# exoplanet-dev/exoplanet

Measured on AMD Instinct MI355X. Metric: light-curve evals/sec (value+grad) at 150k cadences, higher is better.
Workload: dtype f64; 1 GPU; BASELINE configs[1] (C2): single planet e=0.3 Kepler solve + quadratic limb-darkened transit, 150000 cadences, value+grad, use_in_transit=False: dense flux output; n_cadences=150000, draws_per_gpu=1024, global_draws=1024, parallelism=draws sharded over 1 GPU(s); one collective of per-draw scalars per step

## Files before the change

### exoplanet_amd/csrc/exo_transit.hip

```cpp
#include <hip/hip_runtime.h>
#include <stdint.h>

#include "../../include/exoplanet_amd.h"
#include "exo_contact.hpp"
#include "exo_math.hpp"
#include "exo_pack_core.hpp"

namespace {

constexpr int kBlock = 256;
constexpr int kWaves = kBlock / 64;
constexpr int kTile = 2 * kBlock;
#ifndef EXO_TARGET_BLOCKS
#define EXO_TARGET_BLOCKS (256 * 16)
#endif
constexpr int kTargetBlocks = EXO_TARGET_BLOCKS;
constexpr uint32_t kFlagNoFluxDev = 0x80000000u;
constexpr int kNG = 12;
constexpr int kMaxMerge = 8;
constexpr int kWin = 7;
enum { G_N = 0, G_TP, G_ECC, G_COSW, G_SINW, G_COSI, G_AOR, G_ROR, G_FR, G_PAD, G_SINI, G_CL };
constexpr double kCLight = 37231.66360672704;

struct PlanetConst {
  double n, tp, e, se, pe, sq1me2, cw, sw, ci, si, aor, ror, iror;
  double t0, period, iperiod, ts, te, fr, ts2, te2, isq1me2;
  double clr;
  float ef, omf, sqf, cwf, swf, cif, zsf, thrf, zthrf, inthrf;
  double nrev, c0, dmid, half[2];
  double te0, tinv;
  int tfin;
};

struct Shared {
  PlanetConst pc[EXO_MAX_PLANETS];
  double c[6];
  double sdt[EXO_MAX_SUBEXP + 1];
  double sw[EXO_MAX_SUBEXP + 1];
  double red[16][16];
};

#ifndef EXO_WINDOW_REFINE
#define EXO_WINDOW_REFINE 1
#endif
constexpr int kSortBlock = 4096;
constexpr int kWinLanes = 8;
__device__ __forceinline__ void window_lanes(const double* __restrict__ p, uint32_t flags, int sub, double* w) {
  const int which = sub >> 2, k = (sub >> 1) & 1, sd = sub & 1;
  const double e = p[EXO_P_ECC], cw = p[EXO_P_COSW], sw = p[EXO_P_SINW];
  if (flags & EXO_FLAG_WINDOW) {
    const double ip = 1.0 / p[EXO_P_PERIOD];
    const double ts = p[EXO_P_TS], te = p[EXO_P_TE], ts2 = p[EXO_P_TS2], te2 = p[EXO_P_TE2];
    const bool fin = (fabs(ts) < __builtin_inf()) && (fabs(te) < __builtin_inf());
    const bool fin2 = (fabs(ts2) < __builtin_inf()) && (fabs(te2) < __builtin_inf());
    const double mid = fin ? 0.5 * (ts + te) : 0.0, mid2 = fin2 ? 0.5 * (ts2 + te2) : 0.0;
    w[0] = ip;
    w[1] = -(p[EXO_P_T0] + mid) * ip;
    w[2] = (mid - mid2) * ip;
    w[3] = fin ? fma(0.5 * (te - ts) * ip, 1.0 + 1e-12, 1e-14) : __builtin_inf();
    w[4] = fin2 ? fma(0.5 * (te2 - ts2) * ip, 1.0 + 1e-12, 1e-14) : __builtin_inf();
    const double wn_ = sqrt(cw * cw + sw * sw), r_ = fabs(p[EXO_P_ROR]);
    const double sinw_ = wn_ > 0.0 ? sw / wn_ : 0.0;
    for (int q = 0; q < 2; ++q) {
      const double bk = fabs(p[EXO_P_AOR] * p[EXO_P_COSI]) * (1.0 - e * e) / (1.0 + (q ? -e : e) * sinw_);
      const double in2 = (1.0 - r_) * (1.0 - r_) - bk * bk, out2 = (1.0 + r_) * (1.0 + r_) - bk * bk;
      const double h = w[3 + q];
      w[5 + q] = (r_ < 1.0 && in2 > 0.0 && out2 > 0.0 && h < __builtin_inf()) ? 0.95 * h * sqrt(in2 / out2) : 0.0;
    }
    if (flags & EXO_FLAG_LIGHT_DELAY) {
      const double vmax = fabs(p[EXO_P_N] * p[EXO_P_AOR]) * (1.0 + e) / sqrt(1.0 - e * e);
      const double dmax = fabs(p[EXO_P_AOR]) * (1.0 + e) / (fabs(p[EXO_P_CLIGHT]) - vmax);
      const double wd = (dmax >= 0.0 ? dmax : __builtin_inf()) * ip * 1.05;
      w[3] += wd; w[4] += wd;
    }
    return;
  }
  const double nrev = p[EXO_P_N] * (0.5 / exo::kPi);
  const double wn = sqrt(cw * cw + sw * sw);
  const double q = (1.0 + fabs(p[EXO_P_ROR])) / (fabs(p[EXO_P_AOR]) * (1.0 - e) * wn);
  const bool bounded = (e >= 0.0 && e < 1.0) && (q < 0.999);
  const bool want = bounded && (k == 0 || (flags & EXO_FLAG_SECONDARY));
  double m_pt = 0.0;
  bool has_in = false;
  if (want) {
    const double se = sqrt(1.0 - e), pe = sqrt(1.0 + e);
    const double s0 = p[EXO_P_SINI] < 0.0 ? -1.0 : 1.0, sk = k ? -1.0 : 1.0;
    const double sinw = sw / wn, cosw = cw / wn;
// ... 1374 lines not shown
    const double t_rate = (t_last - t_first) / (double)(n_cad > 1 ? n_cad - 1 : 1);
    for (int r = lane; r < K; r += 64) {
      int lo_k = 0, hi_k = nfin + 1;
      while (hi_k - lo_k > 1) {
        const int mid = (lo_k + hi_k) >> 1;
        if (s_first[mid] <= r) lo_k = mid; else hi_k = mid;
      }
      const int k = lo_k;
      const double kc = (double)(s_mlo[k] + (r - s_first[k]));
      const double sh = row.shift[k], off = -sh * nrev;
      auto first_not = [&](double thr, bool strict, int lo, int hi) {
        if (t_rate > 0.0 && hi > lo) {
          const double gq = ceil(((thr - c0) / nrev + sh - t_first) / t_rate);
          const int g = gq < (double)lo ? lo : (gq > (double)hi ? hi : (int)gq);
          const double xa = g > lo ? fma(t[g - 1], nrev, c0) + off : 0.0, xb = g < hi ? fma(t[g], nrev, c0) + off : 0.0;
          const bool left_before = g == lo || (strict ? (xa <= thr) : (xa < thr));
          const bool here_not = g == hi || !(strict ? (xb <= thr) : (xb < thr));
          if (left_before && here_not) return g;
        }
        while (lo < hi) {
          const int mid = (lo + hi) >> 1;
          const double xi = fma(t[mid], nrev, c0) + off;
          const bool before = strict ? (xi <= thr) : (xi < thr);
          lo = before ? mid + 1 : lo;
          hi = before ? hi : mid;
        }
        return lo;
      };
      Run q;
      q.lo = first_not(kc - h0, false, 0, (int)n_cad);
      q.hi = first_not(kc + h0, true, q.lo, (int)n_cad);
      if (hin > 0.0) {
        q.a = first_not(kc - hin, false, q.lo, q.hi);
        q.b = first_not(kc + hin, true, q.a, q.hi);
      } else {
        q.a = q.b = q.lo;
      }
      runs[r] = q;
      rbin[r] = k;
      s_len[0][r] = q.b - q.a;
      s_len[1][r] = q.hi - q.lo;
    }
  }
  __syncthreads();
  enum_prefix(s_len, K, lane, pin, pall, rl.nrun + list);
}

struct FillCursor {
  typedef double v2d __attribute__((ext_vector_type(2)));
  char* base;
  int64_t off;
  int left;
  uint32_t loff;
  v2d zero;
  __device__ __forceinline__ FillCursor(double* dst, int64_t n) : base(nullptr), off(0), left(0), loff((threadIdx.x & 63) * 16) {
    zero = v2d{0.0, 0.0};
    asm volatile("" : "+v"(zero));
    if (!dst || n <= 0) return;
    const int64_t head = (reinterpret_cast<uintptr_t>(dst) & 8) ? 1 : 0;
    if (threadIdx.x == 0 && head) dst[0] = 0.0;
    if (threadIdx.x == 0 && ((n - head) & 1)) dst[n - 1] = 0.0;
    v2d* q2 = reinterpret_cast<v2d*>(dst + head);
    const int64_t n2 = (n - head) >> 1;
    const int64_t nfull = n2 >> 6;
    const int rem = (int)(n2 & 63);
    if ((int)threadIdx.x < rem) __builtin_nontemporal_store(zero, q2 + (nfull << 6) + threadIdx.x);
    const int w = __builtin_amdgcn_readfirstlane((int)(threadIdx.x >> 6));
    left = nfull > w ? (int)((nfull - w + kWaves - 1) / kWaves) : 0;
    left = __builtin_amdgcn_readfirstlane(left);
    base = reinterpret_cast<char*>(q2);
    off = (int64_t)w * 1024;
  }
  __device__ __forceinline__ int pieces_left() const { return left; }
  __device__ __forceinline__ void issue(int count) {
    const int k = count < left ? count : left;
    for (int s = 0; s < k; ++s) {
      __builtin_nontemporal_store(zero, reinterpret_cast<v2d*>(base + off + loff));
      off += kWaves * 1024;
    }
    left -= k;
  }
};

__device__ __forceinline__ void finish_draw(
    int64_t draw, const double* partial, int nblk, int n_planet, bool secondary, double* __restrict__ gparams,
    double* __restrict__ gld, double* __restrict__ flux_dot, int64_t n_cad, uint32_t flags, int n_ev, const RunLists& rl,
    const double* vals, const int32_t* vcad, double* flux,
    const double* __restrict__ chi2_part, int n_chi2_part, double* __restrict__ chi2_out, const Ttv& ttv,
    int64_t cm_draws = 0) {
  if (ttv.gshift) {
    for (int p = 0; p < n_planet; ++p) {
      const int64_t list = draw * n_planet + p;
      const int K = rl.nrun[list];
      const int32_t* __restrict__ rbin = rl.rbin + list * rl.r_max;
      if (K == 0 || rbin[0] < 0) continue;
      const double* grun = rl.grun + list * rl.r_max;
      double* __restrict__ dst = ttv.gshift + list * (int64_t)(ttv.n_edge + 1);
      for (int k = threadIdx.x; k <= ttv.n_edge; k += (int)blockDim.x) {
        int lo = 0, hi = K;
        while (lo < hi) {
          const int mid = (lo + hi) >> 1;
          if (rbin[mid] < k) lo = mid + 1; else hi = mid;
        }
        double v = 0.0;
        for (int r = lo; r < K && rbin[r] == k; ++r) v += grun[r];
        dst[k] = v;
      }
    }
  }
  if (chi2_out && threadIdx.x == blockDim.x - 1) {
    double v = 0.0;
    for (int b = 0; b < n_chi2_part; ++b) v += chi2_part[draw * n_chi2_part + b];
    chi2_out[draw] = v;
  }
  const int ng_draw = n_planet * kNG + 7;
  const int s = threadIdx.x;
  if (partial) {
    for (int q = s; q < n_planet * EXO_NPAR; q += (int)blockDim.x) {
      const int p = q / EXO_NPAR, slot = q % EXO_NPAR;
      const bool carried = slot == EXO_P_N || slot == EXO_P_TP || slot == EXO_P_ECC || slot == EXO_P_COSW ||
                           slot == EXO_P_SINW || slot == EXO_P_COSI || slot == EXO_P_AOR || slot == EXO_P_ROR ||
                           slot == EXO_P_FRATIO || slot == EXO_P_SINI || slot == EXO_P_CLIGHT;
      if (!carried) gparams[(draw * n_planet + p) * EXO_NPAR + slot] = 0.0;
    }
    if (s < ng_draw) {
      const double* src = partial + draw * nblk * (int64_t)ng_draw + s;
      double v = 0.0;
      for (int b = 0; b < nblk; ++b) v += src[(int64_t)b * ng_draw];
      if (s < n_planet * kNG) {
        const int p = s / kNG, k = s % kNG;
        const int map[kNG] = {EXO_P_N, EXO_P_TP, EXO_P_ECC, EXO_P_COSW, EXO_P_SINW,
                              EXO_P_COSI, EXO_P_AOR, EXO_P_ROR, EXO_P_FRATIO, -1, EXO_P_SINI, EXO_P_CLIGHT};
        if (map[k] >= 0) gparams[(draw * n_planet + p) * EXO_NPAR + map[k]] = v;
      } else {
        const int k = s - n_planet * kNG;
        const int nld = secondary ? 6 : 3;
        if (k < nld) gld[draw * nld + k] = v;
        if (k == 6 && flux_dot) flux_dot[draw] = v;
      }
    }
  }
  if (!flux || !vals) return;
  const bool per_planet = flags & EXO_FLAG_PER_PLANET;
  const int nthr = (int)blockDim.x;
  __shared__ int s_total[EXO_MAX_PLANETS];
  if ((int)threadIdx.x < n_planet) {
    int total = 0;
    for (int ev = 0; ev < n_ev; ++ev) {
      const int64_t list = (draw * n_planet + threadIdx.x) * n_ev + ev;
      total += rl.pre_all[list * (rl.r_max + 1) + rl.nrun[list]];
    }
    s_total[threadIdx.x] = total;
  }
  __syncthreads();
  auto total_of = [&](int p) { return s_total[p]; };
  auto load = [&](int p, int cb, int total, double* v, int* i) {
    const int64_t vbase = (draw * n_planet + p) * n_cad;
#pragma unroll
    for (int u = 0; u < 4; ++u) {
      const int e = cb + (int)threadIdx.x + u * nthr;
      v[u] = e < total ? vals[vbase + e] : 0.0;
      i[u] = e < total ? vcad[vbase + e] : -1;
    }
  };
  int pl = 0, cb = -4 * nthr, total = total_of(0);
  auto advance = [&](int& p, int& c, int& tot) {
    c += 4 * nthr;
    while (p < n_planet && c >= tot) {
      ++p; c = 0;
      tot = p < n_planet ? total_of(p) : 0;
    }
  };
  advance(pl, cb, total);
  if (pl >= n_planet) return;
  double v[4];
  int i[4];
  load(pl, cb, total, v, i);
  for (;;) {
    int np = pl, ncb = cb, ntotal = total;
    advance(np, ncb, ntotal);
    const bool more = np < n_planet;
    double nv[4] = {0.0, 0.0, 0.0, 0.0};
    int ni[4] = {-1, -1, -1, -1};
    if (more) load(np, ncb, ntotal, nv, ni);
#pragma unroll
    for (int u = 0; u < 4; ++u) {
      if (i[u] < 0) continue;
      if (per_planet) {
        flux[(draw * n_cad + i[u]) * n_planet + pl] = v[u];
      } else {
        double* dst = cm_draws ? flux + (int64_t)i[u] * cm_draws + draw : flux + draw * n_cad + i[u];
        if (pl == 0) *dst = v[u]; else unsafeAtomicAdd(dst, v[u]);
      }
    }
    if (!more) break;
    if (!per_planet && np != pl) __syncthreads();
    pl = np; cb = ncb; total = ntotal;
#pragma unroll
    for (int u = 0; u < 4; ++u) { v[u] = nv[u]; i[u] = ni[u]; }
  }
}

__global__ __launch_bounds__(1024) void transit_finish_kernel(
    const double* __restrict__ partial, int nblk, int n_planet, bool secondary, double* __restrict__ gparams,
    double* __restrict__ gld, double* __restrict__ flux_dot, int64_t n_cad, uint32_t flags, int n_ev, RunLists rl,
    const double* __restrict__ vals, const int32_t* __restrict__ vcad, double* __restrict__ flux,
    const double* __restrict__ chi2_part, int n_chi2_part, double* __restrict__ chi2_out,
    Ttv ttv = Ttv{nullptr, nullptr, nullptr, 0}) {
  finish_draw(blockIdx.x, partial, nblk, n_planet, secondary, gparams, gld, flux_dot, n_cad, flags, n_ev, rl, vals, vcad, flux,
              chi2_part, n_chi2_part, chi2_out, ttv,
              ((flags & EXO_FLAG_CADENCE_MAJOR) && !(flags & EXO_FLAG_PER_PLANET)) ? (int64_t)gridDim.x : 0);
}

struct FinishArgs {
  double* gparams;
  double* gld;
  double* flux_dot;
  int fold;
  int32_t* done;
};

#ifndef EXO_RUNS_MIN_WAVES
#define EXO_RUNS_MIN_WAVES 3
#endif
constexpr int kJac = 16;
__device__ __forceinline__ int jac_slot(int s) {
  return s < G_PAD ? s : (s == G_SINI ? 9 : (s >= kNG && s < kNG + 6 ? 10 + (s - kNG) : -1));
}
template <bool GRAD, bool SECONDARY, bool LDELAY = false, bool CHI2 = false, bool TTV = false, bool JAC = false>
__global__ __launch_bounds__(kBlock, LDELAY ? 2 : EXO_RUNS_MIN_WAVES) void transit_runs_kernel(
    const double* __restrict__ t, int64_t n_cad, const double* __restrict__ texp, int64_t n_texp,
    const double* __restrict__ stencil_dt, const double* __restrict__ stencil_w, int n_sub,
    const double* __restrict__ params, const double* __restrict__ ld, int n_planet, uint32_t flags, int n_ev, RunLists rl,
    const double* __restrict__ gflux, const double* __restrict__ gsparse, double* __restrict__ vals,
    int32_t* __restrict__ vcad, double* __restrict__ fill, double* __restrict__ partial, int64_t chi2_nw = 0,
    Ttv ttv = Ttv{nullptr, nullptr, nullptr, 0}, FinishArgs fin = FinishArgs{nullptr, nullptr, nullptr, 0, nullptr}) {
  __shared__ Shared sh;
  __shared__ Run s_run[kSeg];
  __shared__ int2 s_pre[kSeg + 1];
  __shared__ int s_all[kSeg + 1];
  __shared__ int s_bin[TTV ? kSeg : 1];
  __shared__ double s_shift[TTV ? kSeg : 1];
  __shared__ double s_grun[(TTV && GRAD) ? kWaves : 1][(TTV && GRAD) ? kSeg : 1];
  __shared__ int s_rounds[2 * EXO_MAX_PLANETS];
  __shared__ double lds_acc[kNG + 7][kBlock];
  const int64_t draw = blockIdx.y;
  const int hb = gridDim.x, bx = blockIdx.x;
  stage_constants(sh, params, ld, stencil_dt, stencil_w, n_sub, n_planet, draw, SECONDARY);
  const bool per_planet = flags & EXO_FLAG_PER_PLANET;
  const int n_lists = n_planet * n_ev;
  auto slice = [&](int K, int& k0, int& k1) {
    k0 = (int)((int64_t)K * bx / hb);
    k1 = (int)((int64_t)K * (bx + 1) / hb);
  };
  if ((int)threadIdx.x < n_lists) {
    const int64_t list = draw * n_lists + threadIdx.x;
    int k0, k1;
    slice(rl.nrun[list], k0, k1);
    const int32_t* pall = rl.pre_all + list * (rl.r_max + 1);
    int rounds = 0;
    for (int kb = k0; kb < k1; kb += kSeg) {
      const int ke = (kb + kSeg < k1) ? kb + kSeg : k1;
      rounds += (pall[ke] - pall[kb] + kBlock - 1) / kBlock;
    }
    s_rounds[threadIdx.x] = rounds;
  }
  __syncthreads();
  int total_rounds = 0;
  for (int l = 0; l < n_lists; ++l) total_rounds += s_rounds[l];
  const int64_t npl = per_planet ? n_planet : 1, n_fill = n_cad * npl;
  const int64_t f0 = n_fill * bx / hb, f1 = n_fill * (bx + 1) / hb;
  FillCursor fc(fill ? fill + draw * n_fill + f0 : nullptr, f1 - f0);
  const int per_round =
      __builtin_amdgcn_readfirstlane(total_rounds > 0 ? (fc.pieces_left() + total_rounds - 1) / total_rounds : 0);

  static_assert(!JAC || (GRAD && !LDELAY && !CHI2 && !TTV), "the Jacobian sweep is the plain value + gradient evaluation");
  const int ng_draw = n_planet * kNG + 7;
  double* __restrict__ pout = (GRAD && !JAC) ? partial + ((int64_t)draw * hb + bx) * ng_draw : nullptr;
  double* __restrict__ jac = JAC ? partial : nullptr;
  const GradAcc acc{GRAD ? &lds_acc[0][threadIdx.x] : nullptr};
  if (GRAD) {
#pragma unroll
    for (int s = 0; s < kNG + 7; ++s) lds_acc[s][threadIdx.x] = 0.0;
  }
  double cld[6];
#pragma unroll
  for (int k = 0; k < 6; ++k) cld[k] = uniform((SECONDARY || k < 3) ? sh.c[k] : 0.0);
  const double te = (n_texp == 0) ? 0.0 : texp[0];
  const double sdt0 = uniform(sh.sdt[0]), sw0 = uniform(sh.sw[0]);
  for (int p = 0; p < n_planet; ++p) {
    const PlanetS c(sh.pc[p]);
    if (GRAD && p > 0) {
#pragma unroll
      for (int s = 0; s < kNG; ++s) lds_acc[s][threadIdx.x] = 0.0;
    }
    int64_t vbase = (draw * n_planet + p) * n_cad;
    const TtvRow row(ttv, TTV ? draw * n_planet + p : 0);
    double* __restrict__ grow = (TTV && GRAD) ? ttv.gshift + (draw * n_planet + p) * (int64_t)(ttv.n_edge + 1) : nullptr;
    const TtvGrad tgrad{(GRAD && TTV) ? &lds_acc[0][threadIdx.x] : nullptr, grow, nullptr};
    for (int ev = 0; ev < n_ev; ++ev) {
      const int64_t list = (draw * n_planet + p) * n_ev + ev;
      const int K = rl.nrun[list];
      const Run* __restrict__ runs = rl.runs + list * rl.r_max;
      const int32_t* __restrict__ pin = rl.pre_in + list * (rl.r_max + 1);
      const int32_t* __restrict__ pall = rl.pre_all + list * (rl.r_max + 1);
      int k0, k1;
      slice(K, k0, k1);
      for (int kb = k0; kb < k1; kb += kSeg) {
        const int m = (kb + kSeg < k1) ? kSeg : k1 - kb;
        __syncthreads();
        const int in0 = pin[kb], all0 = pall[kb];
        for (int q = threadIdx.x; q <= m; q += kBlock) {
          const int pi = pin[kb + q] - in0, pa = pall[kb + q];
          s_pre[q] = make_int2(pi, (pa - all0) - pi);
          s_all[q] = pa;
          if (q < m) s_run[q] = runs[kb + q];
          if (TTV && q < m) {
            const int kq = rl.rbin[list * rl.r_max + kb + q];
            s_bin[q] = kq;
            s_shift[q] = kq >= 0 ? row.shift[kq] : 0.0;
            if (GRAD) {
#pragma unroll
              for (int w = 0; w < kWaves; ++w) s_grun[w][q] = 0.0;
            }
          }
        }
        __syncthreads();
        const bool trusted = TTV && s_bin[0] >= 0;
        const int tin = s_pre[m].x, total = tin + s_pre[m].y;
        const float g_in = tin > 0 ? (float)m / (float)tin : 0.0f;
        const float g_lim = total > tin ? (float)m / (float)(total - tin) : 0.0f;
        struct Item { int i, v, q; double tv, g, w; };
        auto locate = [&](int j, int& i, int& v, int& qrun) {
          const bool in = j < tin;
          const int jj = in ? j : j - tin;
          int q = (int)((float)jj * (in ? g_in : g_lim));
          q = q < m - 1 ? q : m - 1;
          int2 pa = s_pre[q], pb = s_pre[q + 1];
          int lo = in ? pa.x : pa.y, hi = in ? pb.x : pb.y;
          int tries = 0;
          while (EXO_WAVE_ANY((jj < lo) | (jj >= hi))) {
            if (++tries > 4) {
              q = 0;
#pragma unroll
              for (int step = kSeg / 2; step > 0; step >>= 1) {
                const int c2 = q + step;
                if (c2 < m) {
                  const int2 pc = s_pre[c2];
                  q = (jj >= (in ? pc.x : pc.y)) ? c2 : q;
                }
              }
              pa = s_pre[q];
              lo = in ? pa.x : pa.y;
              break;
            }
            q += (jj < lo) ? -1 : ((jj >= hi) ? 1 : 0);
            pa = s_pre[q]; pb = s_pre[q + 1];
            lo = in ? pa.x : pa.y; hi = in ? pb.x : pb.y;
          }
          const Run r = s_run[q];
          const int off = jj - lo;
          i = in ? r.a + off : ((off < r.a - r.lo) ? r.lo + off : r.b + (off - (r.a - r.lo)));
          v = s_all[q] + (i - r.lo);
          qrun = q;
        };
        auto load_item = [&](int j) -> Item {
          Item it{0, 0, 0, 0.0, 0.0, 0.0};
          if (j < total) locate(j, it.i, it.v, it.q);
          it.tv = t[it.i];
          if (JAC) {
            it.g = (j < total) ? 1.0 : 0.0;
          } else if (CHI2) {
            if (j < total) { it.g = gflux[it.i]; it.w = gsparse[chi2_nw == 1 ? 0 : it.i]; }
          } else if (GRAD && j < total)
            it.g = gsparse ? gsparse[vbase + it.v]
                           : (per_planet ? gflux[(draw * n_cad + it.i) * n_planet + p]
                                         : ((flags & EXO_FLAG_CADENCE_MAJOR) ? gflux[(int64_t)it.i * gridDim.y + draw]
                                                                             : gflux[draw * n_cad + it.i]));
          return it;
        };
        Item nxt = load_item(threadIdx.x);
        for (int j0 = 0; j0 < total; j0 += kBlock) {
          const int j = j0 + threadIdx.x;
          const bool has = j < total;
          const Item cur = nxt;
          if (j0 + kBlock < total) nxt = load_item(j + kBlock);
          fc.issue(per_round);
          double f = 0.0;
          const double dsh = TTV ? s_shift[TTV ? cur.q : 0] : 0.0;
          for (int k = 0; k < n_sub; ++k) {
            const double sdt_k = (k == 0) ? sdt0 : sh.sdt[k], sw_k = (k == 0) ? sw0 : sh.sw[k];
            double tt = fma(te, sdt_k, cur.tv);
            int ks = 0;
            if (TTV) {
              double sh_k = dsh;
              if (!trusted) {
                ks = row.bin(tt);
                sh_k = row.shift[ks];
              }
              tt -= sh_k;
            }
            const double gw = cur.g * sw_k;
            const double F = eval_sample<GRAD, SECONDARY, LDELAY, CHI2>(tt, c, cld, CHI2 ? cur.g : gw, acc, cur.w);
            f = fma(sw_k, F, f);
            if (CHI2) {
              const double r = F - cur.g;
              acc.add(kNG + 6, cur.w * (r * r - cur.g * cur.g));
            } else if (GRAD && !JAC) {
              acc.add(kNG + 6, gw * F);
            }
            if (TTV && GRAD && !trusted) tgrad.flush_lane(ks);
          }
          if (TTV && GRAD && trusted) tgrad.flush_runs(cur.q, &s_grun[0][0], kSeg);
          if (JAC) {
            double row[kJac];
#pragma unroll
            for (int q = 0; q < kJac; ++q) row[q] = 0.0;
#pragma unroll
            for (int sl = 0; sl < kNG + 6; ++sl) {
              if (jac_slot(sl) >= 0) {
                row[jac_slot(sl)] = lds_acc[sl][threadIdx.x];
                lds_acc[sl][threadIdx.x] = 0.0;
              }
            }
            if (has) {
              double2* __restrict__ dst = reinterpret_cast<double2*>(jac + (vbase + cur.v) * kJac);
#pragma unroll
              for (int q = 0; q < kJac / 2; ++q) dst[q] = make_double2(row[2 * q], row[2 * q + 1]);
            }
          }
          if (vals && has) {
            vals[vbase + cur.v] = f;
            if (vcad) vcad[vbase + cur.v] = cur.i;
          }
        }
        if (TTV && GRAD && trusted) {
          __syncthreads();
          for (int q = threadIdx.x; q < m; q += kBlock) {
            double v = s_grun[0][q];
#pragma unroll
            for (int w = 1; w < kWaves; ++w) v += s_grun[(TTV && GRAD) ? w : 0][q];
            rl.grun[list * rl.r_max + kb + q] = v;
          }
        }
      }
      vbase += pall[K];
    }
    if (GRAD && TTV) {
      lds_acc[G_TP][threadIdx.x] = lds_acc[G_PAD][threadIdx.x];
      lds_acc[G_PAD][threadIdx.x] = 0.0;
    }
    if (GRAD && !JAC) reduce_columns(lds_acc, sh.red, 0, kNG, pout + p * kNG);
  }
  if (GRAD && !JAC) reduce_columns(lds_acc, sh.red, kNG, 7, pout + n_planet * kNG);
  fc.issue(1 << 30);
  if (fin.fold) {
    __syncthreads();
    finish_draw(draw, (GRAD && !JAC) ? partial : nullptr, hb, n_planet, SECONDARY, fin.gparams, fin.gld, fin.flux_dot, n_cad, flags, n_ev,
                rl, vals, vcad, fill, nullptr, 0, nullptr,
                (TTV && GRAD) ? ttv : Ttv{nullptr, nullptr, nullptr, 0});
  }
}

__global__ __launch_bounds__(kBlock) void transit_jac_vjp_kernel(int64_t n_cad, int n_planet, int n_ev, uint32_t flags,
                                                                 RunLists rl, const double* __restrict__ vals,
                                                                 const int32_t* __restrict__ vcad,
                                                                 const double* __restrict__ jac,
                                                                 const double* __restrict__ gflux, int64_t n_draw,
                                                                 double* __restrict__ partial) {
  __shared__ double red[kJac + 1][kBlock];
  const int64_t draw = blockIdx.y;
  const int nb = gridDim.x, bx = blockIdx.x;
  const int ng_draw = n_planet * kNG + 7;
  double* __restrict__ pout = partial + (draw * nb + bx) * ng_draw;
  const bool cmaj = flags & EXO_FLAG_CADENCE_MAJOR, gsp = flags & EXO_FLAG_SPARSE;
  double keep = 0.0;
  for (int p = 0; p < n_planet; ++p) {
    int n_vals = 0;
    for (int ev = 0; ev < n_ev; ++ev) {
      const int64_t list = (draw * n_planet + p) * n_ev + ev;
      n_vals += rl.pre_all[list * (rl.r_max + 1) + rl.nrun[list]];
    }
    const int64_t vbase = (draw * n_planet + p) * n_cad;
    double acc[kJac + 1];
#pragma unroll
    for (int q = 0; q <= kJac; ++q) acc[q] = 0.0;
    const int v0 = (int)((int64_t)n_vals * bx / nb), v1 = (int)((int64_t)n_vals * (bx + 1) / nb);
    for (int v = v0 + threadIdx.x; v < v1; v += kBlock) {
      double g;
      if (gsp) {
        g = gflux[vbase + v];
      } else {
        const int64_t i = vcad[vbase + v];
        g = cmaj ? gflux[i * n_draw + draw] : gflux[draw * n_cad + i];
      }
      const double2* __restrict__ row = reinterpret_cast<const double2*>(jac + (vbase + v) * kJac);
#pragma unroll
      for (int q = 0; q < kJac / 2; ++q) {
        const double2 r2 = row[q];
        acc[2 * q] = fma(g, r2.x, acc[2 * q]);
        acc[2 * q + 1] = fma(g, r2.y, acc[2 * q + 1]);
      }
      acc[kJac] = fma(g, vals[vbase + v], acc[kJac]);
    }
    __syncthreads();
#pragma unroll
    for (int q = 0; q <= kJac; ++q) red[q][threadIdx.x] = acc[q];
    __syncthreads();
    if (threadIdx.x <= kJac) {
      double v = 0.0;
      for (int k = 0; k < kBlock; ++k) v += red[threadIdx.x][k];
      const int q = threadIdx.x;
      if (q < 10) {
        pout[p * kNG + (q < 9 ? q : G_SINI)] = v;
      } else {
        keep += v;
      }
    }
    if (threadIdx.x < kNG && (threadIdx.x == G_PAD || threadIdx.x == G_CL)) pout[p * kNG + threadIdx.x] = 0.0;
  }
  if (threadIdx.x >= 10 && threadIdx.x <= kJac) pout[n_planet * kNG + (threadIdx.x - 10)] = keep;
}

constexpr int kResidualBlocks = 16;
__global__ __launch_bounds__(kBlock) void transit_residual_kernel(int64_t n_cad, int n_planet, int n_ev, RunLists rl,
                                                                  const double* __restrict__ vals,
                                                                  const int32_t* __restrict__ vcad,
                                                                  const double* __restrict__ obs,
                                                                  const double* __restrict__ ivar, int64_t n_ivar,
                                                                  double* __restrict__ gvals,
                                                                  double* __restrict__ chi2_part) {
  __shared__ double red[kBlock];
  const int64_t draw = blockIdx.y;
  const int nb = gridDim.x, n_lists = n_planet * n_ev;
  double acc = 0.0;
  auto lookup = [&](int l2, int i, bool& hit) -> double {
    const int64_t list = draw * n_lists + l2;
    const int K = rl.nrun[list];
    const Run* __restrict__ runs = rl.runs + list * rl.r_max;
    int lo = 0, hi = K;
    while (lo < hi) {
      const int mid = (lo + hi) >> 1;
// ... 118 lines not shown
  int64_t n_classify;
  dim3 grid;
};
inline ScanPlan scan_plan(uint32_t flags, int bpd, int64_t n_draw, int n_planet, int64_t n_texp, bool with_fill) {
  ScanPlan sp;
  const bool stage1 = (flags & EXO_FLAG_WINDOW) || !(flags & EXO_FLAG_EXACT_SCAN);
  const bool grouped = n_planet == 1 && n_texp <= 1 && stage1;
  sp.flags = (flags & 0x0fffffffu) | (grouped ? kFlagGrouped : 0u) | (with_fill ? 0u : kFlagNoFlux);
  sp.n_classify = (grouped ? (n_draw + kScanDraws - 1) / kScanDraws : n_draw) * bpd;
  sp.grid = dim3((unsigned)(sp.n_classify + (with_fill ? n_draw * bpd : 0)));
  return sp;
}

#ifndef EXO_RUNS_TARGET_BLOCKS
#define EXO_RUNS_TARGET_BLOCKS 512
#endif
inline int runs_blocks_per_draw(int64_t n_draw) {
  int64_t hb = (EXO_RUNS_TARGET_BLOCKS + n_draw - 1) / n_draw;
  return (int)(hb < 1 ? 1 : (hb > 64 ? 64 : hb));
}
inline int runs_r_max(int64_t n_cad) { return (int)(n_cad < kRunMax ? (n_cad < 16 ? 16 : n_cad) : kRunMax); }

struct RunWs {
  double* partial;
  double* windows;
  int32_t* sorted;
  RunLists rl;
  double* vals;
  int32_t* vcad;
  double* gvals;
  double* chi2_part;
  int32_t* done;
  int hb, n_sorted;
  int64_t off_nrun, off_runs, off_pre_all, off_vals;
  int64_t bytes;
};
inline RunWs carve_runs(void* base, int64_t n_cad, int64_t n_draw, int n_planet) {
  RunWs w;
  w.hb = runs_blocks_per_draw(n_draw);
  w.n_sorted = (int)((n_cad + kSortBlock - 1) / kSortBlock);
  w.rl.r_max = runs_r_max(n_cad);
  const int64_t n_list = n_draw * n_planet * 2;
  auto up16 = [](int64_t b) { return (b + 15) & ~(int64_t)15; };
  char* p = (char*)base;
  int64_t off = 0;
  w.partial = (double*)(p + off); off = up16(off + 8 * n_draw * w.hb * (int64_t)(n_planet * kNG + 7));
  w.windows = (double*)(p + off); off = up16(off + 8 * (int64_t)kWin * n_draw * n_planet);
  w.sorted = (int32_t*)(p + off); off = up16(off + 4 * (int64_t)w.n_sorted);
  w.off_nrun = off; w.rl.nrun = (int32_t*)(p + off); off = up16(off + 4 * n_list);
  w.off_runs = off; w.rl.runs = (Run*)(p + off); off = up16(off + (int64_t)sizeof(Run) * n_list * w.rl.r_max);
  w.rl.pre_in = (int32_t*)(p + off); off = up16(off + 4 * n_list * (int64_t)(w.rl.r_max + 1));
  w.off_pre_all = off; w.rl.pre_all = (int32_t*)(p + off); off = up16(off + 4 * n_list * (int64_t)(w.rl.r_max + 1));
  w.rl.rbin = (int32_t*)(p + off); off = up16(off + 4 * n_draw * n_planet * (int64_t)w.rl.r_max);
  w.rl.grun = (double*)(p + off); off = up16(off + 8 * n_draw * n_planet * (int64_t)w.rl.r_max);
  w.off_vals = off; w.vals = (double*)(p + off); off = up16(off + 8 * n_draw * n_planet * n_cad);
  w.vcad = (int32_t*)(p + off); off = up16(off + 4 * n_draw * n_planet * n_cad);
  w.gvals = (double*)(p + off); off = up16(off + 8 * n_draw * n_planet * n_cad);
  w.chi2_part = (double*)(p + off); off = up16(off + 8 * n_draw * kResidualBlocks);
  w.done = (int32_t*)(p + off); off = up16(off + 4 * n_draw);
  w.bytes = off;
  return w;
}
inline bool runs_path(bool has_ttv, int64_t n_texp, uint32_t flags) {
  if (has_ttv && (flags & (EXO_FLAG_SECONDARY | EXO_FLAG_LIGHT_DELAY))) return false;
  return n_texp <= 1 && !(flags & EXO_FLAG_EXACT_SCAN);
}

struct Chi2Args {
  const double* obs;
  const double* ivar;
  int64_t n_ivar;
  double* chi2;
};
struct RunsCommon {
  dim3 grid;
  hipStream_t st;
  const double *t, *texp, *stencil_dt, *stencil_w, *params, *ld;
  int64_t n_cad, n_texp;
  int n_sub, n_planet, n_ev;
  uint32_t flags;
  RunLists rl;
  Ttv ttv;
};
template <bool G, bool SEC, bool LDELAY = false, bool CHI2 = false, bool TTV = false, bool JAC = false>
inline void launch_runs(const RunsCommon& a, const double* gflux, const double* gsparse, double* vals, int32_t* vcad, double* fill,
                        double* partial, const FinishArgs& fin, int64_t chi2_nw = 0) {
  hipLaunchKernelGGL((transit_runs_kernel<G, SEC, LDELAY, CHI2, TTV, JAC>), a.grid, dim3(kBlock), 0, a.st, a.t, a.n_cad, a.texp,
                     a.n_texp, a.stencil_dt, a.stencil_w, a.n_sub, a.params, a.ld, a.n_planet, a.flags, a.n_ev, a.rl, gflux, gsparse,
                     vals, vcad, fill, partial, chi2_nw, a.ttv, fin);
}
inline int launch_runs_sweep(const double* t, int64_t n_cad, const double* texp, int64_t n_texp, const double* stencil_dt,
                             const double* stencil_w, int32_t n_sub, const double* params, const double* ld,
                             int64_t n_draw, int32_t n_planet, uint32_t flags, const double* gflux, double* flux,
                             double* gparams, double* gld, double* flux_dot, const RunWs& w, hipStream_t st,
                             const Chi2Args* chi2 = nullptr, const Ttv* ttv = nullptr, double* jac = nullptr,
                             const double* gvals = nullptr, bool reuse_runs = false, const PackIn* pack = nullptr) {
  const bool secondary = flags & EXO_FLAG_SECONDARY, sparse = (flags & EXO_FLAG_SPARSE) || chi2;
  const bool grad = gflux != nullptr || chi2 || gvals != nullptr;
  const int n_ev = secondary ? 2 : 1;
  const dim3 block(kBlock);
  const bool has_ttv = ttv && ttv->edges;
  const bool fused_enum = (flags & EXO_FLAG_SORTED_TIMES) && !has_ttv;
  if (reuse_runs) {
  } else if (!fused_enum) {
    const int64_t n_rec = n_draw * n_planet;
    hipLaunchKernelGGL(transit_window_kernel, dim3((unsigned)((n_rec * kWinLanes + kBlock - 1) / kBlock + w.n_sorted)), block, 0, st,
                       params, n_rec, flags, w.windows, t, n_cad, w.sorted, w.done, n_draw);
  }
  if (pack && (!fused_enum || reuse_runs)) return EXO_ERR_INVALID_ARGUMENT;
  if (reuse_runs) {
  } else if (pack) {
    const PackIn pk = *pack;
    hipLaunchKernelGGL((transit_enum_kernel<true, true>), dim3((unsigned)(n_draw * n_planet * n_ev)), dim3(64), 0, st, t, n_cad, texp,
                       n_texp, stencil_dt, (int)n_sub, flags, (const double*)nullptr, (const int32_t*)nullptr, 0, n_ev, w.rl,
                       params, w.windows, pk);
  } else if (fused_enum)
    hipLaunchKernelGGL(transit_enum_kernel<true>, dim3((unsigned)(n_draw * n_planet * n_ev)), dim3(64), 0, st, t, n_cad, texp,
                       n_texp, stencil_dt, (int)n_sub, flags, (const double*)nullptr, (const int32_t*)nullptr, 0, n_ev, w.rl,
                       params, w.windows);
  else if (has_ttv)
    hipLaunchKernelGGL(transit_enum_ttv_kernel, dim3((unsigned)(n_draw * n_planet)), dim3(64), 0, st, t, n_cad, texp, n_texp,
                       stencil_dt, (int)n_sub, flags, w.windows, w.sorted, w.n_sorted, w.rl, *ttv);
  else
    hipLaunchKernelGGL(transit_enum_kernel<false>, dim3((unsigned)(n_draw * n_planet * n_ev)), dim3(64), 0, st, t, n_cad, texp,
                       n_texp, stencil_dt, (int)n_sub, flags, w.windows, w.sorted, w.n_sorted, n_ev, w.rl);
  if (launch_status() != EXO_OK) return EXO_ERR_LAUNCH;
  double* vals = (flux || sparse) ? w.vals : nullptr;
  double* fill = sparse ? nullptr : flux;
  const bool ldelay = flags & EXO_FLAG_LIGHT_DELAY;
  const Ttv no_ttv{nullptr, nullptr, nullptr, 0};
  const RunsCommon ra{dim3((unsigned)w.hb, (unsigned)n_draw), st, t, texp, stencil_dt, stencil_w, params, ld, n_cad, n_texp, (int)n_sub,
                      (int)n_planet, n_ev, flags, w.rl, has_ttv ? *ttv : no_ttv};
  const bool cmaj = flags & EXO_FLAG_CADENCE_MAJOR;
  const bool fold = !(cmaj && flux) && w.hb == 1;
  const FinishArgs fin{gparams, gld, chi2 ? chi2->chi2 : flux_dot, fold ? 1 : 0, w.done}, no_fin{nullptr, nullptr, nullptr, 0, nullptr};
  auto plain = [&](auto g, const double* gf, const double* gsp, double* v, int32_t* vc, double* fl, double* part, const FinishArgs& f) {
    exo::with_flag(secondary, [&](auto sec) {
      exo::with_flag(ldelay, [&](auto ldl) {
        launch_runs<decltype(g)::value, decltype(sec)::value, decltype(ldl)::value>(ra, gf, gsp, v, vc, fl, part, f);
      });
    });
  };
  if (chi2 && n_planet == 1 && !secondary && n_sub == 1) {
    if (has_ttv)
      launch_runs<true, false, false, true, true>(ra, chi2->obs, chi2->ivar, nullptr, nullptr, nullptr, w.partial, fin, chi2->n_ivar);
    else if (ldelay)
      launch_runs<true, false, true, true>(ra, chi2->obs, chi2->ivar, nullptr, nullptr, nullptr, w.partial, fin, chi2->n_ivar);
    else
      launch_runs<true, false, false, true>(ra, chi2->obs, chi2->ivar, nullptr, nullptr, nullptr, w.partial, fin, chi2->n_ivar);
    if (launch_status() != EXO_OK) return EXO_ERR_LAUNCH;
    if (fold) return EXO_OK;
    hipLaunchKernelGGL(transit_finish_kernel, dim3((unsigned)n_draw), dim3(n_draw <= 256 ? 1024 : kBlock), 0, st, w.partial, w.hb,
                       (int)n_planet, secondary, gparams, gld, chi2->chi2, n_cad, flags, n_ev, w.rl, nullptr, w.vcad, nullptr,
                       nullptr, 0, nullptr, ra.ttv);
    return launch_status();
  }
  if (has_ttv && chi2) {
    launch_runs<false, false, false, false, true>(ra, nullptr, nullptr, w.vals, w.vcad, nullptr, nullptr, no_fin);
    hipLaunchKernelGGL(transit_residual_kernel, dim3(kResidualBlocks, (unsigned)n_draw), block, 0, st, n_cad, (int)n_planet,
                       n_ev, w.rl, w.vals, w.vcad, chi2->obs, chi2->ivar, chi2->n_ivar, w.gvals, w.chi2_part);
    launch_runs<true, false, false, false, true>(ra, nullptr, w.gvals, nullptr, nullptr, nullptr, w.partial, no_fin);
  } else if (has_ttv) {
    if (grad)
      launch_runs<true, false, false, false, true>(ra, gflux, nullptr, vals, fill ? w.vcad : nullptr, fill, w.partial, fin);
    else
      launch_runs<false, false, false, false, true>(ra, nullptr, nullptr, vals, fill ? w.vcad : nullptr, fill, nullptr, fin);
  } else if (chi2) {
    plain(std::false_type{}, nullptr, nullptr, w.vals, w.vcad, nullptr, nullptr, no_fin);
    hipLaunchKernelGGL(transit_residual_kernel, dim3(kResidualBlocks, (unsigned)n_draw), block, 0, st, n_cad, (int)n_planet,
                       n_ev, w.rl, w.vals, w.vcad, chi2->obs, chi2->ivar, chi2->n_ivar, w.gvals, w.chi2_part);
    plain(std::true_type{}, nullptr, w.gvals, nullptr, nullptr, nullptr, w.partial, no_fin);
  } else if (gvals) {
    plain(std::true_type{}, nullptr, gvals, nullptr, nullptr, nullptr, w.partial, fin);
  } else if (grad) {
    plain(std::true_type{}, gflux, nullptr, vals, fill ? w.vcad : nullptr, fill, w.partial, fin);
  } else if (jac) {
    exo::with_flag(secondary, [&](auto sec) {
      launch_runs<true, decltype(sec)::value, false, false, false, true>(ra, nullptr, nullptr, vals, w.vcad, fill, jac, fin);
    });
  } else {
    plain(std::false_type{}, nullptr, nullptr, vals, fill ? w.vcad : nullptr, fill, nullptr, fin);
  }
  if (launch_status() != EXO_OK) return EXO_ERR_LAUNCH;
  const bool three_sweeps = chi2 != nullptr;
  if ((grad || fill) && (!fold || three_sweeps))
    hipLaunchKernelGGL(transit_finish_kernel, dim3((unsigned)n_draw), dim3(n_draw <= 256 ? 1024 : kBlock), 0, st,
                       grad ? w.partial : nullptr, w.hb, (int)n_planet, secondary, gparams, gld, flux_dot, n_cad, flags, n_ev,
                       w.rl, chi2 ? nullptr : vals, w.vcad, fill, chi2 ? w.chi2_part : nullptr, kResidualBlocks,
                       chi2 ? chi2->chi2 : nullptr, grad ? ra.ttv : no_ttv);
  return launch_status();
}

template <bool CLEAR>
__global__ __launch_bounds__(kBlock) void transit_scatter_runs_kernel(RunLists rl, const double* __restrict__ vals, int64_t n_cad,
                                                                      int n_planet, int n_ev, double* __restrict__ flux) {
  const int64_t draw = blockIdx.x;
  const int wave = threadIdx.x >> 6, lane = threadIdx.x & 63, n_wave = kBlock / 64;
  double* __restrict__ row = flux + draw * n_cad;
  for (int p = 0; p < n_planet; ++p) {
    int64_t vbase = (draw * n_planet + p) * n_cad;
    for (int ev = 0; ev < n_ev; ++ev) {
      const int64_t list = (draw * n_planet + p) * n_ev + ev;
      int K = rl.nrun[list];
      K = K < 0 ? 0 : (K > rl.r_max ? rl.r_max : K);
      const Run* __restrict__ runs = rl.runs + list * rl.r_max;
      const int32_t* __restrict__ pall = rl.pre_all + list * (rl.r_max + 1);
      for (int k = wave; k < K; k += n_wave) {
        int lo = runs[k].lo, len = runs[k].hi - lo;
        const int pk = pall[k];
        if (lo < 0 || len < 0 || (int64_t)lo + len > n_cad || pk < 0 || (int64_t)pk + len > n_cad) continue;
        const int64_t v0 = vbase + pk;
        for (int i = lane; i < len; i += 64) {
          if (CLEAR) row[lo + i] = 0.0;
          else if (p == 0) row[lo + i] = vals[v0 + i];
          else unsafeAtomicAdd(row + lo + i, vals[v0 + i]);
        }
      }
      const int tot = pall[K];
      vbase += (tot < 0 || tot > n_cad) ? 0 : tot;
    }
    if (!CLEAR && p + 1 < n_planet) __syncthreads();
  }
}

struct MergeWs {
  int32_t* nseg;
  int32_t* seg;
  int32_t* off;
  int32_t* sorted;
  double* vals;
  int cap_seg, cap_run;
  int64_t off_nseg, off_seg, off_off, off_vals, bytes;
};
inline MergeWs carve_merge(void* base, int64_t n_cad, int64_t n_draw, int n_planet) {
  MergeWs m;
  const int64_t runs = (int64_t)n_planet * 2 * runs_r_max(n_cad);
  m.cap_run = (int)runs;
  m.cap_seg = (int)(runs < n_cad + 1 ? runs : n_cad + 1);
  auto up16 = [](int64_t b) { return (b + 15) & ~(int64_t)15; };
  char* p = (char*)base;
  int64_t off = 0;
  m.off_nseg = off; m.nseg = (int32_t*)(p + off); off = up16(off + 4 * n_draw);
  m.off_seg = off; m.seg = (int32_t*)(p + off); off = up16(off + 8 * n_draw * (int64_t)m.cap_seg);
  m.off_off = off; m.off = (int32_t*)(p + off); off = up16(off + 4 * n_draw * ((int64_t)m.cap_seg + 1));
  m.sorted = (int32_t*)(p + off); off = up16(off + 8 * n_draw * (int64_t)m.cap_run);
  m.off_vals = off; m.vals = (double*)(p + off); off = up16(off + 8 * n_draw * n_cad);
  m.bytes = off;
  return m;
}
inline int merge_blocks_per_draw(int64_t n_draw) {
  const int64_t b = (4096 + n_draw - 1) / (n_draw > 0 ? n_draw : 1);
  return (int)(b < 1 ? 1 : (b > 64 ? 64 : b));
}

__device__ __forceinline__ int runs_lower(const Run* __restrict__ runs, int K, int key, bool or_equal) {
  int lo = 0, hi = K;
  while (lo < hi) {
    const int mid = (lo + hi) >> 1;
    const int v = runs[mid].lo;
    if (v < key || (or_equal && v == key)) lo = mid + 1; else hi = mid;
  }
  return lo;
}
__device__ __forceinline__ int runs_find(const Run* __restrict__ runs, int K, int n) {
  const int k = runs_lower(runs, K, n, true) - 1;
  return (k >= 0 && n < runs[k].hi) ? k : -1;
}

// ... 669 lines not shown
```

Baseline: 3.729 million evals/s.

## Write single-planet transit flux in place and zero-fill only gaps between runs

For the plain single-planet dense-flux case, the runs kernel now writes each in-transit flux value straight into the output row. A new gap-aware fill cursor zeroes only the 128-cadence pieces not covered by transit runs, using per-lane masks on partial pieces. Before, values went to a sparse buffer with cadence indices, the whole row was zeroed, and the finish kernel scattered the values back. Removing that buffer and the scatter saves global traffic and work in the finish step, at the cost of run-list lookups and masked stores inside the fill loop.

```diff
diff --git a/exoplanet_amd/csrc/exo_fill_core.hpp b/exoplanet_amd/csrc/exo_fill_core.hpp
--- /dev/null
+++ b/exoplanet_amd/csrc/exo_fill_core.hpp
@@ -0,0 +1,85 @@
+#pragma once
+#include <stdint.h>
+
+#if defined(__HIPCC__)
+#define EXO_FILL_HD __host__ __device__ __forceinline__
+#else
+#define EXO_FILL_HD inline
+#endif
+
+namespace exo_fill {
+
+constexpr int kPiece = 128;
+
+struct Share {
+  int64_t f0, f1;
+  int64_t c0, c1;
+  int a0;
+};
+
+EXO_FILL_HD Share make_share(int64_t n_cad, int bx, int hb, int a0) {
+  Share s;
+  s.f0 = n_cad * bx / hb;
+  s.f1 = n_cad * (bx + 1) / hb;
+  s.a0 = a0;
+  s.c0 = (s.f0 + a0) >> 7;
+  s.c1 = s.f1 > s.f0 ? ((s.f1 + a0 + kPiece - 1) >> 7) : s.c0;
+  return s;
+}
+EXO_FILL_HD int64_t piece_lo(const Share& s, int64_t c) { return (c << 7) - s.a0; }
+
+EXO_FILL_HD int wave_pieces(const Share& s, int w, int n_wave) {
+  const int64_t n = s.c1 - s.c0;
+  return n > w ? (int)((n - w + n_wave - 1) / n_wave) : 0;
+}
+
+struct RunCursor {
+  int k, K;
+  int32_t lo, hi;
+  template <class Runs>
+  EXO_FILL_HD void load(const Runs& runs) {
+    lo = k < K ? runs.lo(k) : 0;
+    hi = k < K ? runs.hi(k) : 0;
+  }
+  template <class Runs>
+  EXO_FILL_HD void start(const Runs& runs, int n_run, int64_t p0) {
+    K = n_run;
+    int a = 0, b = n_run;
+    while (a < b) {
+      const int mid = (a + b) >> 1;
+      if (runs.hi(mid) <= p0) a = mid + 1; else b = mid;
+    }
+    k = a;
+    load(runs);
+  }
+  template <class Runs>
+  EXO_FILL_HD void advance(const Runs& runs, int64_t p0) {
+    while (k < K && (hi <= p0 || hi <= lo)) {
+      ++k;
+      load(runs);
+    }
+  }
+};
+
+enum Kind { kWhole = 0, kCovered = 1, kMasked = 2 };
+EXO_FILL_HD int classify(const Share& s, int64_t p0, const RunCursor& rc) {
+  const int64_t p1 = p0 + kPiece;
+  const bool has_run = rc.k < rc.K;
+  if (has_run && rc.lo <= p0 && rc.hi >= p1) return kCovered;
+  const bool inside = p0 >= s.f0 && p1 <= s.f1;
+  return (inside && (!has_run || rc.lo >= p1)) ? kWhole : kMasked;
+}
+
+template <class Runs>
+EXO_FILL_HD int lane_mask(const Share& s, const Runs& runs, int K, int k, int64_t p0, int lane) {
+  const int64_t e = p0 + 2 * lane, p1 = p0 + kPiece;
+  bool z0 = e >= s.f0 && e < s.f1, z1 = e + 1 >= s.f0 && e + 1 < s.f1;
+  for (int j = k; j < K && runs.lo(j) < p1; ++j) {
+    const int64_t lo = runs.lo(j), hi = runs.hi(j);
+    z0 = z0 && !(e >= lo && e < hi);
+    z1 = z1 && !(e + 1 >= lo && e + 1 < hi);
+  }
+  return (z0 ? 1 : 0) | (z1 ? 2 : 0);
+}
+
+}
diff --git a/exoplanet_amd/csrc/exo_transit.hip b/exoplanet_amd/csrc/exo_transit.hip
--- a/exoplanet_amd/csrc/exo_transit.hip
+++ b/exoplanet_amd/csrc/exo_transit.hip
@@ -3,6 +3,7 @@
 
 #include "../../include/exoplanet_amd.h"
 #include "exo_contact.hpp"
+#include "exo_fill_core.hpp"
 #include "exo_math.hpp"
 #include "exo_pack_core.hpp"
 
@@ -1543,6 +1544,54 @@
   }
 };
 
+struct GapCursor {
+  typedef double v2d __attribute__((ext_vector_type(2)));
+  struct RunsView {
+    const Run* __restrict__ r;
+    __device__ __forceinline__ int32_t lo(int k) const { return __builtin_amdgcn_readfirstlane(r[k].lo); }
+    __device__ __forceinline__ int32_t hi(int k) const { return __builtin_amdgcn_readfirstlane(r[k].hi); }
+  };
+  char* base;
+  exo_fill::Share s;
+  exo_fill::RunCursor rc;
+  RunsView view;
+  int64_t c;
+  int left;
+  int lane;
+  v2d zero;
+  __device__ __forceinline__ GapCursor(double* row, int64_t n_cad, int bx, int hb, const Run* runs, int K)
+      : view{runs}, lane(threadIdx.x & 63) {
+    zero = v2d{0.0, 0.0};
+    asm volatile("" : "+v"(zero));
+    const int a0 = (int)((reinterpret_cast<uintptr_t>(row) >> 3) & 1);
+    s = exo_fill::make_share(n_cad, bx, hb, a0);
+    base = reinterpret_cast<char*>(row) - 8 * a0;
+    const int w = __builtin_amdgcn_readfirstlane((int)(threadIdx.x >> 6));
+    left = __builtin_amdgcn_readfirstlane(exo_fill::wave_pieces(s, w, kWaves));
+    c = s.c0 + w;
+    rc.start(view, __builtin_amdgcn_readfirstlane(K), exo_fill::piece_lo(s, c));
+  }
+  __device__ __forceinline__ int pieces_left() const { return left; }
+  __device__ __forceinline__ void issue(int count) {
+    const int n = count < left ? count : left;
+    for (int q = 0; q < n; ++q, c += kWaves) {
+      const int64_t p0 = exo_fill::piece_lo(s, c);
+      rc.advance(view, p0);
+      const int kind = exo_fill::classify(s, p0, rc);
+      if (kind == exo_fill::kWhole) {
+        __builtin_nontemporal_store(zero, reinterpret_cast<v2d*>(base + (c << 10) + (uint32_t)(lane * 16)));
+      } else if (kind == exo_fill::kMasked) {
+        const int m = exo_fill::lane_mask(s, view, rc.K, rc.k, p0, lane);
+        double* q2 = reinterpret_cast<double*>(base + (c << 10) + (uint32_t)(lane * 16));
+        if (m == 3) *reinterpret_cast<v2d*>(q2) = zero;
+        else if (m == 1) q2[0] = 0.0;
+        else if (m == 2) q2[1] = 0.0;
+      }
+    }
+    left -= n;
+  }
+};
+
 __device__ __forceinline__ void finish_draw(
     int64_t draw, const double* partial, int nblk, int n_planet, bool secondary, double* __restrict__ gparams,
     double* __restrict__ gld, double* __restrict__ flux_dot, int64_t n_cad, uint32_t flags, int n_ev, const RunLists& rl,
@@ -1688,7 +1737,7 @@
 __device__ __forceinline__ int jac_slot(int s) {
   return s < G_PAD ? s : (s == G_SINI ? 9 : (s >= kNG && s < kNG + 6 ? 10 + (s - kNG) : -1));
 }
-template <bool GRAD, bool SECONDARY, bool LDELAY = false, bool CHI2 = false, bool TTV = false, bool JAC = false>
+template <bool GRAD, bool SECONDARY, bool LDELAY = false, bool CHI2 = false, bool TTV = false, bool JAC = false, bool INPLACE = false>
 __global__ __launch_bounds__(kBlock, LDELAY ? 2 : EXO_RUNS_MIN_WAVES) void transit_runs_kernel(
     const double* __restrict__ t, int64_t n_cad, const double* __restrict__ texp, int64_t n_texp,
     const double* __restrict__ stencil_dt, const double* __restrict__ stencil_w, int n_sub,
@@ -1731,7 +1780,13 @@
   for (int l = 0; l < n_lists; ++l) total_rounds += s_rounds[l];
   const int64_t npl = per_planet ? n_planet : 1, n_fill = n_cad * npl;
   const int64_t f0 = n_fill * bx / hb, f1 = n_fill * (bx + 1) / hb;
-  FillCursor fc(fill ? fill + draw * n_fill + f0 : nullptr, f1 - f0);
+  static_assert(!INPLACE || (!SECONDARY && !CHI2 && !TTV && !JAC), "in-place values: one list per draw, plain sweep");
+  auto fc = [&] {
+    if constexpr (INPLACE)
+      return GapCursor(fill + draw * n_cad, n_cad, bx, hb, rl.runs + draw * rl.r_max, rl.nrun[draw]);
+    else
+      return FillCursor(fill ? fill + draw * n_fill + f0 : nullptr, f1 - f0);
+  }();
   const int per_round =
       __builtin_amdgcn_readfirstlane(total_rounds > 0 ? (fc.pieces_left() + total_rounds - 1) / total_rounds : 0);
 
@@ -1890,7 +1945,9 @@
               for (int q = 0; q < kJac / 2; ++q) dst[q] = make_double2(row[2 * q], row[2 * q + 1]);
             }
           }
-          if (vals && has) {
+          if (INPLACE) {
+            if (has) fill[draw * n_cad + cur.i] = f;
+          } else if (vals && has) {
             vals[vbase + cur.v] = f;
             if (vcad) vcad[vbase + cur.v] = cur.i;
           }
@@ -1918,7 +1975,7 @@
   if (fin.fold) {
     __syncthreads();
     finish_draw(draw, (GRAD && !JAC) ? partial : nullptr, hb, n_planet, SECONDARY, fin.gparams, fin.gld, fin.flux_dot, n_cad, flags, n_ev,
-                rl, vals, vcad, fill, nullptr, 0, nullptr,
+                rl, INPLACE ? nullptr : vals, INPLACE ? nullptr : vcad, INPLACE ? nullptr : fill, nullptr, 0, nullptr,
                 (TTV && GRAD) ? ttv : Ttv{nullptr, nullptr, nullptr, 0});
   }
 }
@@ -2203,10 +2260,10 @@
   RunLists rl;
   Ttv ttv;
 };
-template <bool G, bool SEC, bool LDELAY = false, bool CHI2 = false, bool TTV = false, bool JAC = false>
+template <bool G, bool SEC, bool LDELAY = false, bool CHI2 = false, bool TTV = false, bool JAC = false, bool INPLACE = false>
 inline void launch_runs(const RunsCommon& a, const double* gflux, const double* gsparse, double* vals, int32_t* vcad, double* fill,
                         double* partial, const FinishArgs& fin, int64_t chi2_nw = 0) {
-  hipLaunchKernelGGL((transit_runs_kernel<G, SEC, LDELAY, CHI2, TTV, JAC>), a.grid, dim3(kBlock), 0, a.st, a.t, a.n_cad, a.texp,
+  hipLaunchKernelGGL((transit_runs_kernel<G, SEC, LDELAY, CHI2, TTV, JAC, INPLACE>), a.grid, dim3(kBlock), 0, a.st, a.t, a.n_cad, a.texp,
                      a.n_texp, a.stencil_dt, a.stencil_w, a.n_sub, a.params, a.ld, a.n_planet, a.flags, a.n_ev, a.rl, gflux, gsparse,
                      vals, vcad, fill, partial, chi2_nw, a.ttv, fin);
 }
@@ -2246,8 +2303,10 @@
     hipLaunchKernelGGL(transit_enum_kernel<false>, dim3((unsigned)(n_draw * n_planet * n_ev)), dim3(64), 0, st, t, n_cad, texp,
                        n_texp, stencil_dt, (int)n_sub, flags, w.windows, w.sorted, w.n_sorted, n_ev, w.rl);
   if (launch_status() != EXO_OK) return EXO_ERR_LAUNCH;
-  double* vals = (flux || sparse) ? w.vals : nullptr;
   double* fill = sparse ? nullptr : flux;
+  const bool inplace = fill && n_planet == 1 && !secondary && !has_ttv && !jac && !chi2 && !gvals &&
+                       !(flags & (EXO_FLAG_CADENCE_MAJOR | EXO_FLAG_PER_PLANET));
+  double* vals = (!inplace && (flux || sparse)) ? w.vals : nullptr;
   const bool ldelay = flags & EXO_FLAG_LIGHT_DELAY;
   const Ttv no_ttv{nullptr, nullptr, nullptr, 0};
   const RunsCommon ra{dim3((unsigned)w.hb, (unsigned)n_draw), st, t, texp, stencil_dt, stencil_w, params, ld, n_cad, n_texp, (int)n_sub,
@@ -2260,6 +2319,12 @@
       exo::with_flag(ldelay, [&](auto ldl) {
         launch_runs<decltype(g)::value, decltype(sec)::value, decltype(ldl)::value>(ra, gf, gsp, v, vc, fl, part, f);
       });
+    });
+  };
+  auto plain_inplace = [&](auto g, const double* gf, double* part) {
+    exo::with_flag(ldelay, [&](auto ldl) {
+      launch_runs<decltype(g)::value, false, decltype(ldl)::value, false, false, false, true>(ra, gf, nullptr, nullptr, nullptr, fill,
+                                                                                              part, fin);
     });
   };
   if (chi2 && n_planet == 1 && !secondary && n_sub == 1) {
@@ -2293,6 +2358,9 @@
     plain(std::true_type{}, nullptr, w.gvals, nullptr, nullptr, nullptr, w.partial, no_fin);
   } else if (gvals) {
     plain(std::true_type{}, nullptr, gvals, nullptr, nullptr, nullptr, w.partial, fin);
+  } else if (inplace) {
+    if (grad) plain_inplace(std::true_type{}, gflux, w.partial);
+    else plain_inplace(std::false_type{}, nullptr, nullptr);
   } else if (grad) {
     plain(std::true_type{}, gflux, nullptr, vals, fill ? w.vcad : nullptr, fill, w.partial, fin);
   } else if (jac) {
@@ -2304,7 +2372,7 @@
   }
   if (launch_status() != EXO_OK) return EXO_ERR_LAUNCH;
   const bool three_sweeps = chi2 != nullptr;
-  if ((grad || fill) && (!fold || three_sweeps))
+  if ((grad || (fill && !inplace)) && (!fold || three_sweeps))
     hipLaunchKernelGGL(transit_finish_kernel, dim3((unsigned)n_draw), dim3(n_draw <= 256 ? 1024 : kBlock), 0, st,
                        grad ? w.partial : nullptr, w.hb, (int)n_planet, secondary, gparams, gld, flux_dot, n_cad, flags, n_ev,
                        w.rl, chi2 ? nullptr : vals, w.vcad, fill, chi2 ? w.chi2_part : nullptr, kResidualBlocks,
```

Result: slower. 2.881 million evals/s (-22.7%).
